# lambdaji/tf_repos

Hardware: NVIDIA H100
Metric: DeepFM training samples/sec, Criteo-39-field synthetic (39 fields, 200M vocab, k=16, bs=8192) (higher is better)
Workload: dtype f32

## Files before the change

include/ctr_b200.h:

```cpp
#ifndef CTR_B200_H_
#define CTR_B200_H_

#include <stddef.h>
#include <stdint.h>

#ifdef __cplusplus
extern "C" {
#endif

typedef void* ctr_stream_t;

enum ctr_status {
  CTR_OK = 0,
  CTR_ERR_INVALID_ARG = -1,
  CTR_ERR_UNSUPPORTED = -2,
  CTR_ERR_CUDA = -3,
  CTR_ERR_WORKSPACE = -4
};

enum ctr_fm_mode {
  CTR_FM_DEEPFM = 0,
  CTR_FM_NFM = 1,
  CTR_FM_PLAIN = 2
};
// ... 65 lines not shown
int ctr_epoch_sweep(int opt, float* var, float* slot0, float* slot1, uint8_t* last, int64_t n_rows, int K,
                    const float* hyper, const float* lr_table, int from, int upto, int reset, double* ss_partials,
                    int* n_partials_host, int32_t* list, int64_t list_cap, int32_t* list_count, double* ss_rows,
                    ctr_stream_t stream);
int ctr_epoch_sweep_ovf(int opt, float* var, float* slot0, float* slot1, uint8_t* last, int64_t n_rows, int K,
                        const float* hyper, const float* lr_table, int from, int upto, int reset, double* ss_partials,
                        int* n_partials_host, int32_t* list, int64_t list_cap, int32_t* list_count, double* ss_rows,
                        int32_t* list_overflow, ctr_stream_t stream);
int ctr_epoch_sweep2_supported(int opt, int64_t n_rows, int K);
int ctr_epoch_sweep2(int opt, float* var, float* slot0, float* slot1, float* w_var, float* w_slot0, float* w_slot1,
                     uint8_t* last, int64_t n_rows, int K, const float* hyper, const float* lr_table, int from, int upto,
                     int reset, double* ss_partials, double* w_ss_partials, int* n_partials_host, int32_t* list,
                     int64_t list_cap, int32_t* list_count, double* ss_rows, double* w_ss_rows, int32_t* list_overflow,
                     ctr_stream_t stream);
int ctr_epoch_reg_loss(double* ss_rows, const double* ss_partials, int n_partials, int upto, float scale,
                       float* reg, int accumulate, ctr_stream_t stream);
int ctr_selftest_divsqrt(uint64_t seed, int64_t n, int64_t* mismatches, ctr_stream_t stream);
int ctr_selftest_adam_packed(int regime, uint64_t seed, int64_t n, int steps, float lr, float l2, int64_t* out3,
                             ctr_stream_t stream);

int ctr_logit_loss(const float* bias, const float* y_a, const float* y_b, const float* y_c,
                   const float* labels, int B, int B_total, float* y, float* pred, float* loss_ce,
                   float* dy, float* dbias, ctr_stream_t stream);

int ctr_fc_fwd(const float* in, const float* Wt, const float* b, const float* drop_mask, float keep_prob,
               int M, int Kd, int Nd, int act, float* out, ctr_stream_t stream);
int ctr_fc_fwd_grouped(const float* in, const float* Wt, const float* b, const float* group_bias, int group_P,
                       const float* drop_mask, float keep_prob, int M, int Kd, int Nd, int act, float* out,
                       ctr_stream_t stream);
size_t ctr_fc_bwd_workspace_bytes(int M, int Kd, int Nd);
int ctr_fc_bwd(const float* in, const float* Wt, const float* out, const float* drop_mask, float keep_prob,
               float* dOut, int M, int Kd, int Nd, int act, float* dIn, int accumulate_din, float* dW, float* db,
               void* ws, size_t ws_bytes, ctr_stream_t stream);
int ctr_fc1_fwd(const float* in_a, int Ka, const float* in_b, int Kb, const float* w, const float* b, int M,
                float* y, ctr_stream_t stream);
size_t ctr_fc1_bwd_workspace_bytes(int M, int Ka, int Kb);
int ctr_fc1_bwd(const float* in_a, int Ka, const float* in_b, int Kb, const float* w, const float* dy, int M,
                float* d_a, float* d_b, float* dw, float* db, void* ws, size_t ws_bytes, ctr_stream_t stream);
int ctr_dropout_mask(float* mask, int64_t n, float keep_prob, uint64_t seed, const float* step_dev,
                     ctr_stream_t stream);

size_t ctr_bn_workspace_bytes(int H);
int ctr_bn_fwd(const float* x, int n, int H, const float* gamma, const float* beta, float* moving_mean,
               float* moving_var, int train, float decay, float eps, const float* drop_mask, float keep_prob, float* out,
               float* save_mean, float* save_var, void* ws, size_t ws_bytes, ctr_stream_t stream);
int ctr_bn_bwd(const float* d_out, const float* x, int n, int H, const float* save_mean, const float* save_var,
               const float* gamma, float eps, const float* drop_mask, float keep_prob, float* d_x, float* d_gamma,
               float* d_beta, void* ws, size_t ws_bytes, ctr_stream_t stream);

int ctr_cross_fwd(const float* x0, const float* w, const float* b, int B, int D, int L, float* xL, float* s,
                  ctr_stream_t stream);
size_t ctr_cross_bwd_workspace_bytes(int B, int D, int L);
int ctr_cross_bwd(const float* x0, const float* w, const float* b, const float* s, const float* dxL,
                  const float* dx_in, int B, int D, int L, float* dx0, float* dw, float* db, void* ws,
                  size_t ws_bytes, ctr_stream_t stream);

int ctr_mvm_fwd(const float* x, const float* mvm_b, int B, int F, int K, float* x_mvm, ctr_stream_t stream);
size_t ctr_mvm_bwd_workspace_bytes(int B, int F, int K);
int ctr_mvm_bwd(const float* x, const float* mvm_b, const float* d_xmvm, const float* dX, int B, int F, int K,
                float* d_e, float* d_mvm_b, void* ws, size_t ws_bytes, ctr_stream_t stream);

int ctr_esmm_embed_fwd(const int32_t* feat_ids, const int32_t* a_ids, const int32_t* bag_ids, const float* bag_wgt,
                       const int32_t* bag_off, const float* V, int64_t N, int B, int Fp, int K, float* x, int32_t* oob,
                       ctr_stream_t stream);
int ctr_esmm_embed_bwd(const float* dx, const float* bag_wgt, const int32_t* bag_off, int B, int Fp, int K,
                       int64_t n_rows, float* g_rows, ctr_stream_t stream);
// ... 145 lines not shown
```

tf_repos_b200/_lib.py:

```python
from __future__ import annotations

import ctypes
import os
from ctypes import c_char_p, c_float, c_int, c_int32, c_int64, c_size_t, c_uint64, c_void_p

_HERE = os.path.dirname(os.path.abspath(__file__))
LIB_PATH = os.path.join(_HERE, "libctr_b200.so")


class CtrError(RuntimeError):
    pass


def _load() -> ctypes.CDLL:
    if not os.path.exists(LIB_PATH):
        raise CtrError(
            f"{LIB_PATH} not found: build it with `make` (or `python -c 'import __graft_entry__ as g; "
            "g.build()'`). There is no CPU/eager fallback for the hot path."
        )
    return ctypes.CDLL(LIB_PATH)


_lib = _load()

# ... 7 lines not shown
    "ctr_fm_embed_bwd": (c_int, [P, P, P, P, P, P, c_int, c_int, c_int, c_int, P, P, P]),
    "ctr_unique_segment_workspace_bytes": (c_size_t, [c_int64, c_int64]),
    "ctr_unique_segment": (c_int, [P, c_int64, c_int64, P, P, P, P, P, P, P, c_size_t, P]),
    "ctr_segment_sum_rows": (c_int, [P, P, P, P, P, P, c_int64, c_int, P, P, P, c_size_t, P]),
    "ctr_opt_sparse_rows": (c_int, [c_int, P, P, P, P, P, P, c_int64, c_int, P, P, P]),
    "ctr_opt_dense_sweep": (c_int, [c_int, P, P, P, c_int64, P, P, ctypes.POINTER(c_int), P]),
    "ctr_opt_patch_rows": (c_int, [P, P, P, P, P, P, c_int64, c_int, c_int, P]),
    "ctr_opt_dense_grad": (c_int, [c_int, P, P, P, P, c_int64, P, P]),
    "ctr_adam_tick": (c_int, [P, P, c_int, P]),
    "ctr_epoch_max_steps": (c_int, []),
    "ctr_epoch_tick": (c_int, [P, P, c_int, P, c_int, c_int, P]),
    "ctr_epoch_rows": (c_int, [c_int, c_int, P, P, P, P, P, P, P, c_int64, c_int, P, P, c_int, P, P]),
    "ctr_epoch_rows2": (c_int, [c_int, c_int, P, P, P, P, P, P, P, P, P, P, P, P, c_int64, c_int, P, P, c_int, P, P, P]),
    "ctr_epoch_rows2_staged": (c_int, [c_int, c_int, P, P, P, P, P, P, P, P, P, P, P, P, c_int64, c_int, P, P, c_int, P,
                                       P, P, P, P]),
    "ctr_epoch_sweep": (c_int, [c_int, P, P, P, P, c_int64, c_int, P, P, c_int, c_int, c_int, P,
                                ctypes.POINTER(c_int), P, c_int64, P, P, P]),
    "ctr_epoch_sweep_ovf": (c_int, [c_int, P, P, P, P, c_int64, c_int, P, P, c_int, c_int, c_int, P,
                                    ctypes.POINTER(c_int), P, c_int64, P, P, P, P]),
    "ctr_epoch_sweep2_supported": (c_int, [c_int, c_int64, c_int]),
    "ctr_epoch_sweep2": (c_int, [c_int, P, P, P, P, P, P, P, c_int64, c_int, P, P, c_int, c_int, c_int, P, P,
                                 ctypes.POINTER(c_int), P, c_int64, P, P, P, P, P]),
    "ctr_epoch_reg_loss": (c_int, [P, P, c_int, c_int, c_float, P, c_int, P]),
    "ctr_selftest_divsqrt": (c_int, [c_uint64, c_int64, P, P]),
    "ctr_selftest_adam_packed": (c_int, [c_int, c_uint64, c_int64, c_int, c_float, c_float, P, P]),
    "ctr_reduce_sum": (c_int, [P, c_int64, c_float, P, P, c_size_t, P]),
    "ctr_l2_loss_workspace_bytes": (c_size_t, [c_int64]),
    "ctr_l2_loss": (c_int, [P, c_int64, c_float, P, P, c_size_t, P]),
    "ctr_logit_loss": (c_int, [P, P, P, P, P, c_int, c_int, P, P, P, P, P, P]),
    "ctr_fc_fwd": (c_int, [P, P, P, P, c_float, c_int, c_int, c_int, c_int, P, P]),
    "ctr_fc_bwd_workspace_bytes": (c_size_t, [c_int, c_int, c_int]),
    "ctr_fc_fwd_grouped": (c_int, [P, P, P, P, c_int, P, c_float, c_int, c_int, c_int, c_int, P, P]),
    "ctr_fc_bwd": (c_int, [P, P, P, P, c_float, P, c_int, c_int, c_int, c_int, P, c_int, P, P, P, c_size_t, P]),
    "ctr_fc1_fwd": (c_int, [P, c_int, P, c_int, P, P, c_int, P, P]),
    "ctr_fc1_bwd_workspace_bytes": (c_size_t, [c_int, c_int, c_int]),
    "ctr_fc1_bwd": (c_int, [P, c_int, P, c_int, P, P, c_int, P, P, P, P, P, c_size_t, P]),
    "ctr_dropout_mask": (c_int, [P, c_int64, c_float, c_uint64, P, P]),
    "ctr_bn_workspace_bytes": (c_size_t, [c_int]),
    "ctr_bn_fwd": (c_int, [P, c_int, c_int, P, P, P, P, c_int, c_float, c_float, P, c_float, P, P, P, P, c_size_t, P]),
    "ctr_bn_bwd": (c_int, [P, P, c_int, c_int, P, P, P, c_float, P, c_float, P, P, P, P, c_size_t, P]),
    "ctr_cross_fwd": (c_int, [P, P, P, c_int, c_int, c_int, P, P, P]),
    "ctr_cross_bwd_workspace_bytes": (c_size_t, [c_int, c_int, c_int]),
    "ctr_cross_bwd": (c_int, [P, P, P, P, P, P, c_int, c_int, c_int, P, P, P, P, c_size_t, P]),
    "ctr_mvm_fwd": (c_int, [P, P, c_int, c_int, c_int, P, P]),
    "ctr_mvm_bwd_workspace_bytes": (c_size_t, [c_int, c_int, c_int]),
    "ctr_mvm_bwd": (c_int, [P, P, P, P, c_int, c_int, c_int, P, P, P, c_size_t, P]),
    "ctr_esmm_embed_fwd": (c_int, [P, P, P, P, P, P, c_int64, c_int, c_int, c_int, P, P, P]),
    "ctr_esmm_embed_bwd": (c_int, [P, P, P, c_int, c_int, c_int, c_int64, P, P]),
    "ctr_esmm_head": (c_int, [P, P, P, P, c_int, c_int, c_float, c_float, P, P, P, P, P, P, P]),
    "ctr_gather_scale_rows": (c_int, [P, P, P, c_int64, c_int64, c_int, c_int, c_int64, P, P, P]),
    "ctr_bag_sum_fwd": (c_int, [P, P, P, P, c_int64, c_int, c_int, c_int64, P, P]),
    "ctr_bag_sum_fwd_oob": (c_int, [P, P, P, P, c_int64, c_int, c_int, c_int64, P, P, P]),
    "ctr_bag_sum_bwd": (c_int, [P, c_int64, P, P, c_int, c_int, P, P]),
    "ctr_scale_rows": (c_int, [P, P, P, c_int64, c_int, c_int, c_int64, P, P]),
    "ctr_din_pool_fwd": (c_int, [P, P, P, c_int, c_int, c_int, P, P, c_int64, P]),
    "ctr_din_pool_bwd": (c_int, [P, P, P, P, c_int64, c_int, c_int, c_int, P, P, P]),
    "ctr_group_sum": (c_int, [P, c_int, c_int, c_int, P, P]),
    "ctr_din_att_dz": (c_int, [P, P, c_float, P, P, c_int, c_int, c_int, P, P, P, P]),
    "ctr_colsum_rows": (c_int, [P, c_int, c_int, c_int, P, P]),
    "ctr_axpby": (c_int, [P, c_float, P, c_float, c_int64, P, P]),
    "ctr_pnn_product_fwd": (c_int, [P, c_int, c_int, c_int, c_int, P, P]),
    "ctr_pnn_product_bwd": (c_int, [P, P, c_int, c_int, c_int, c_int, P, P]),
    "ctr_afm_pairs_fwd": (c_int, [P, c_int, c_int, c_int, P, P]),
    "ctr_afm_pairs_bwd": (c_int, [P, P, c_int, c_int, c_int, P, P]),
    "ctr_afm_pool_fwd": (c_int, [P, P, P, c_float, c_int, c_int, c_int, P, P, P]),
    "ctr_afm_pool_bwd": (c_int, [P, P, P, c_float, P, c_int, c_int, c_int, P, P, P]),
# ... 77 lines not shown
```

tf_repos_b200/base.py:

```python
from __future__ import annotations

from typing import Dict, List, Optional

import torch

from . import ops
from .engine import DenseVars, OptimizerState, SparseModel, SparseUpdater, Table


def ints(s) -> List[int]:
    return [int(t) for t in s.split(",")] if isinstance(s, str) else list(s)


def floats(s) -> List[float]:
    return [float(t) for t in s.split(",")] if isinstance(s, str) else list(s)


class CTRModel(SparseModel):
    replayed_launches = 0
    batch_norm, bn_decay = False, 0.9
    table_name = "emb"
    linear_name: Optional[str] = None

    def __init__(self, field_size: int, feature_size: int, embedding_size: int, batch_size: int,
# ... 58 lines not shown
        B = ids.shape[0]
        self.flush()
        bias, y_a, y_b, y_c = self._forward(ids, vals, train=False)
        ops.logit_loss(bias, y_a, y_b, y_c, None, B, y=self.y[:B], pred=self.pred[:B])
        return self.pred[:B]

    def train_step(self, ids: torch.Tensor, vals: torch.Tensor, labels: torch.Tensor, masks=None) -> torch.Tensor:
        B, F, K = ids.shape[0], self.F, self.K
        assert B <= self.B, "batch larger than the configured batch_size"
        assert B == self.B or self.world == 1, "partial batches are not supported under data parallelism"
        deferred = self.update_mode == "exact_deferred"
        upd = self.updater
        upd.begin_step()
        ids_u = ids.reshape(-1)
        if deferred and self.world > 1:
            import torch.distributed as dist
            dist.all_gather_into_tensor(self.ids_all, ids_u)
            ids_u = self.ids_all
        upd.catch_up(ids_u)
        bias, y_a, y_b, y_c = self._forward(ids, vals, train=True, masks=masks)
        ops.logit_loss(bias, y_a, y_b, y_c, labels, B, y=self.y[:B], pred=self.pred[:B], loss_ce=self.loss_ce,
                       dy=self.dy[:B], dbias=(self.dense.grads[self.bias_name] if self.bias_name else None),
                       B_total=B * self.world)
        self._backward(ids, vals)
        g_rows = self.g_rows[: B * F]
        g_w = self.g_w[: B * F] if self.g_w is not None else None
        if self.world > 1:
            import torch.distributed as dist
            if not deferred:
                dist.all_gather_into_tensor(self.ids_all, ids.reshape(-1))
            dist.all_gather_into_tensor(self.g_rows_all, g_rows)
            if g_w is not None:
                dist.all_gather_into_tensor(self.g_w_all, g_w)
            dist.all_reduce(self.dense.grad)
            g_rows, g_w = self.g_rows_all, (self.g_w_all if g_w is not None else None)
        upd.finish_step(self.ids_all if self.world > 1 else ids.reshape(-1), g_rows, g_w)
        dense_reg = self._dense_reg_terms()
        self.dense.apply()
        self.global_step += 1
        parts = [self.loss_ce]
        if dense_reg is not None and not self.table_reg_first:
            parts.append(dense_reg)
        if self.W is not None:
            parts.append(upd.reg[1:2])
        parts.append(upd.reg[0:1])
        if dense_reg is not None and self.table_reg_first:
            parts.append(dense_reg)
        return torch.cat(parts)

    bias_name: Optional[str] = None
    table_reg_first = False

    def train_step_graphed(self, ids: torch.Tensor, vals: torch.Tensor, labels: torch.Tensor) -> torch.Tensor:
        B = ids.shape[0]
        deferred = self.update_mode == "exact_deferred"
        ends_epoch = deferred and self.epoch_pos == self.epoch_steps - 1
        if B != self.B or self.world != 1 or ends_epoch:
            return self.train_step(ids, vals, labels)
        if not hasattr(self, "_graphs"):
            self._graphs, self._graph_out, self._graph_seen = {}, {}, {}
            self._gin = (torch.empty(self.B, self.F, dtype=torch.int32, device=self.device),
                         torch.empty(self.B, self.F, dtype=torch.float32, device=self.device),
                         torch.empty(self.B, dtype=torch.float32, device=self.device))
        for dst, src in zip(self._gin, (ids, vals, labels)):
            dst.copy_(src, non_blocking=True)
        key = (self.update_mode, self.epoch_pos if deferred else 0)
# ... 50 lines not shown
```

tf_repos_b200/csrc/fc.cu:

```cuda
#include <stdlib.h>
#include <string.h>

#include "common.cuh"

namespace ctr {

constexpr int GEMM_BK = 16;

template <int BM, int BN, int TM, int TN, bool A_RC, bool B_RC, int EPI>
__global__ void __launch_bounds__((BM / TM) * (BN / TN))
gemm_tile_kernel(const float* __restrict__ A, int lda, const float* __restrict__ B, int ldb,
                 float* __restrict__ C, int ldc, int M, int N, int R, const float* __restrict__ bias,
                 int act, const float* __restrict__ mask, float keep, const float* __restrict__ gbias,
                 int gP) {
  constexpr int NT = (BM / TM) * (BN / TN);
  __shared__ __align__(16) float As[2][GEMM_BK][BM + 4];
  __shared__ __align__(16) float Bs[2][GEMM_BK][BN + 4];
  const int tid = threadIdx.x;
  const int tx = tid % (BN / TN), ty = tid / (BN / TN);
  const int i0 = blockIdx.y * BM, j0 = blockIdx.x * BN;
  const int r_chunk = (R + gridDim.z - 1) / gridDim.z;
  const int r_begin = blockIdx.z * r_chunk;
  const int r_end = min(R, r_begin + r_chunk);

// ... 228 lines not shown
int ctr_fc_fwd_grouped(const float* in, const float* Wt, const float* b, const float* group_bias, int group_P,
                       const float* drop_mask, float keep_prob, int M, int Kd, int Nd, int act, float* out,
                       ctr_stream_t stream);

int ctr_fc_fwd(const float* in, const float* Wt, const float* b, const float* drop_mask, float keep_prob,
               int M, int Kd, int Nd, int act, float* out, ctr_stream_t stream) {
  return ctr_fc_fwd_grouped(in, Wt, b, nullptr, 1, drop_mask, keep_prob, M, Kd, Nd, act, out, stream);
}

int ctr_fc_fwd_grouped(const float* in, const float* Wt, const float* b, const float* group_bias, int group_P,
                       const float* drop_mask, float keep_prob, int M, int Kd, int Nd, int act, float* out,
                       ctr_stream_t stream) {
  CTR_REQUIRE(M >= 0 && Kd > 0 && Nd > 0 && (act == 0 || act == 1) && group_P >= 1, CTR_ERR_INVALID_ARG,
              "ctr_fc_fwd: bad shape/act");
  if (M == 0) return CTR_OK;
  CTR_REQUIRE(in && Wt && out, CTR_ERR_INVALID_ARG, "ctr_fc_fwd: null buffer");
  CTR_REQUIRE(!drop_mask || keep_prob > 0.f, CTR_ERR_INVALID_ARG, "ctr_fc_fwd: keep_prob must be > 0");
  cudaStream_t st = as_stream(stream);
  if (use_tc()) {
    tc_gemm_dispatch(0, 1, in, Kd, Wt, Nd, out, Nd, M, Nd, Kd, 1, b, act, drop_mask, keep_prob, group_bias, group_P, st);
  } else if (Nd >= 128) {
    dim3 grid((Nd + 127) / 128, (M + 63) / 64, 1);
    gemm_tile_kernel<64, 128, 4, 8, true, false, 1><<<grid, 256, 0, st>>>(in, Kd, Wt, Nd, out, Nd, M, Nd, Kd, b, act,
                                                                          drop_mask, keep_prob, group_bias, group_P);
  } else {
    dim3 grid((Nd + 63) / 64, (M + 63) / 64, 1);
    gemm_tile_kernel<64, 64, 4, 4, true, false, 1><<<grid, 256, 0, st>>>(in, Kd, Wt, Nd, out, Nd, M, Nd, Kd, b, act,
                                                                         drop_mask, keep_prob, group_bias, group_P);
  }
  CTR_LAUNCHED("ctr_fc_fwd");
  return CTR_OK;
}

size_t ctr_fc_bwd_workspace_bytes(int M, int Kd, int Nd) {
  if (M <= 0 || Kd <= 0 || Nd <= 0) return 0;
  const size_t chunks = (size_t)(M + DZ_ROWS - 1) / DZ_ROWS;
  const size_t split = 64;
  return (chunks * (size_t)Nd + split * (size_t)Kd * (size_t)Nd) * sizeof(float);
}

int ctr_fc_bwd(const float* in, const float* Wt, const float* out, const float* drop_mask, float keep_prob,
               float* dOut, int M, int Kd, int Nd, int act, float* dIn, int accumulate_din, float* dW, float* db,
               void* ws, size_t ws_bytes, ctr_stream_t stream) {
  CTR_REQUIRE(M >= 0 && Kd > 0 && Nd > 0 && (act == 0 || act == 1 || act == 2), CTR_ERR_INVALID_ARG, "ctr_fc_bwd: bad shape/act");
  if (M == 0) return CTR_OK;
  CTR_REQUIRE(in && Wt && dOut && dW && (act == 2 || (out && db)), CTR_ERR_INVALID_ARG, "ctr_fc_bwd: null buffer");
  CTR_REQUIRE(ws && ws_bytes >= ctr_fc_bwd_workspace_bytes(M, Kd, Nd), CTR_ERR_WORKSPACE,
              "ctr_fc_bwd: workspace too small");
  cudaStream_t st = as_stream(stream);
  float* colsum = reinterpret_cast<float*>(ws);
  const int chunks = (M + DZ_ROWS - 1) / DZ_ROWS;
  float* dw_part = colsum + (size_t)chunks * Nd;
  if (act != 2) {
    fc_dz_kernel<<<dim3((Nd + 31) / 32, chunks), 256, 0, st>>>(dOut, out, drop_mask, keep_prob, M, Nd, act, colsum);
    CTR_LAUNCHED("fc_dz");
    colsum_rows_kernel<<<(Nd + 31) / 32, 256, 0, st>>>(colsum, chunks, Nd, Nd, Nd, db, nullptr);
    CTR_LAUNCHED("fc_db_reduce");
  }
  const bool dw_transposed = use_tc() && Kd <= 64 && Nd >= 128;
  const int S = dw_transposed ? pick_split(Nd, Kd, M) : pick_split(Kd, Nd, M);
  if (dw_transposed) {
    tc_gemm_dispatch(2, 0, dOut, Nd, in, Kd, dw_part, Kd, Nd, Kd, M, S, nullptr, 0, nullptr, 1.f, nullptr, 1, st);
    CTR_LAUNCHED("fc_dw(t)");
    const int64_t n = (int64_t)Kd * Nd;
    splitk_reduce_t_kernel<<<(unsigned)((n + 255) / 256), 256, 0, st>>>(dw_part, S, Kd, Nd, dW);
    CTR_LAUNCHED("fc_dw_reduce(t)");
  } else {
    if (use_tc()) {
      tc_gemm_dispatch(2, 0, in, Kd, dOut, Nd, S == 1 ? dW : dw_part, Nd, Kd, Nd, M, S, nullptr, 0, nullptr, 1.f, nullptr, 1, st);
    } else {
      dim3 grid((Nd + 63) / 64, (Kd + 63) / 64, S);
      gemm_tile_kernel<64, 64, 4, 4, false, false, 0><<<grid, 256, 0, st>>>(in, Kd, dOut, Nd, S == 1 ? dW : dw_part, Nd,
                                                                            Kd, Nd, M, nullptr, 0, nullptr, 1.f, nullptr, 1);
    }
    CTR_LAUNCHED("fc_dw");
    if (S > 1) {
      const int64_t n = (int64_t)Kd * Nd;
      splitk_reduce_kernel<<<(unsigned)((n + 255) / 256), 256, 0, st>>>(dw_part, S, n, dW);
      CTR_LAUNCHED("fc_dw_reduce");
    }
  }
  if (dIn && use_tc()) {
    tc_gemm_dispatch(1, accumulate_din ? 2 : 0, dOut, Nd, Wt, Nd, dIn, Kd, M, Kd, Nd, 1, nullptr, 0, nullptr, 1.f, nullptr, 1, st);
    CTR_LAUNCHED("fc_din");
  } else if (dIn) {
    dim3 grid((Kd + 127) / 128, (M + 63) / 64, 1);
    if (accumulate_din)
      gemm_tile_kernel<64, 128, 4, 8, true, true, 2><<<grid, 256, 0, st>>>(dOut, Nd, Wt, Nd, dIn, Kd, M, Kd, Nd, nullptr,
                                                                           0, nullptr, 1.f, nullptr, 1);
    else
      gemm_tile_kernel<64, 128, 4, 8, true, true, 0><<<grid, 256, 0, st>>>(dOut, Nd, Wt, Nd, dIn, Kd, M, Kd, Nd, nullptr,
                                                                           0, nullptr, 1.f, nullptr, 1);
    CTR_LAUNCHED("fc_din");
  }
  return CTR_OK;
}

int ctr_colsum_rows(const float* part, int rows, int ld, int ncols, float* out, ctr_stream_t stream) {
  CTR_REQUIRE(rows >= 0 && ncols > 0 && ld >= ncols, CTR_ERR_INVALID_ARG, "ctr_colsum_rows: bad shape");
  CTR_REQUIRE(part && out, CTR_ERR_INVALID_ARG, "ctr_colsum_rows: null buffer");
  colsum_rows_kernel<<<(ncols + 31) / 32, 256, 0, as_stream(stream)>>>(part, rows, ld, ncols, ncols, out, nullptr);
  CTR_LAUNCHED("ctr_colsum_rows");
  return CTR_OK;
}

int ctr_fc1_fwd(const float* in_a, int Ka, const float* in_b, int Kb, const float* w, const float* b, int M,
                float* y, ctr_stream_t stream) {
  CTR_REQUIRE(M >= 0 && Ka > 0 && Kb >= 0, CTR_ERR_INVALID_ARG, "ctr_fc1_fwd: bad shape");
  if (M == 0) return CTR_OK;
  CTR_REQUIRE(in_a && w && y && (Kb == 0 || in_b), CTR_ERR_INVALID_ARG, "ctr_fc1_fwd: null buffer");
  fc1_fwd_kernel<<<(M + 7) / 8, 256, 0, as_stream(stream)>>>(in_a, Ka, in_b, Kb, w, b, M, y);
  CTR_LAUNCHED("ctr_fc1_fwd");
  return CTR_OK;
}

size_t ctr_fc1_bwd_workspace_bytes(int M, int Ka, int Kb) {
  if (M <= 0) return 0;
  return (size_t)((M + FC1_ROWS - 1) / FC1_ROWS) * (size_t)(Ka + Kb + 1) * sizeof(float);
}

int ctr_fc1_bwd(const float* in_a, int Ka, const float* in_b, int Kb, const float* w, const float* dy, int M,
                float* d_a, float* d_b, float* dw, float* db, void* ws, size_t ws_bytes, ctr_stream_t stream) {
  CTR_REQUIRE(M >= 0 && Ka > 0 && Kb >= 0, CTR_ERR_INVALID_ARG, "ctr_fc1_bwd: bad shape");
  if (M == 0) return CTR_OK;
  CTR_REQUIRE(in_a && w && dy && dw && db && (Kb == 0 || in_b), CTR_ERR_INVALID_ARG, "ctr_fc1_bwd: null buffer");
  CTR_REQUIRE(ws && ws_bytes >= ctr_fc1_bwd_workspace_bytes(M, Ka, Kb), CTR_ERR_WORKSPACE,
              "ctr_fc1_bwd: workspace too small");
  cudaStream_t st = as_stream(stream);
  const int chunks = (M + FC1_ROWS - 1) / FC1_ROWS;
  float* part = reinterpret_cast<float*>(ws);
// ... 22 lines not shown
```

tf_repos_b200/deepfm.py:

```python
from __future__ import annotations

import torch

from . import ops
from .base import CTRModel, floats, ints
from .engine import DenseVars
from .mlp import MLP


class DeepFM(CTRModel):
    table_name = "fm_v"
    linear_name = "fm_w"
    bias_name = "fm_bias"

    def __init__(self, field_size: int, feature_size: int, embedding_size: int, batch_size: int,
                 deep_layers="256,128,64", dropout="0.5,0.5,0.5", l2_reg: float = 1e-4,
                 learning_rate: float = 5e-4, optimizer: str = "Adam", update_mode: str = "exact",
                 device="cuda", seed: int = 0, world: int = 1, epoch_steps: int = 8, batch_norm: bool = False,
                 batch_norm_decay: float = 0.9):
        self.layers, self.keep = ints(deep_layers), floats(dropout)
        self.batch_norm, self.bn_decay = bool(batch_norm), float(batch_norm_decay)
        super().__init__(field_size, feature_size, embedding_size, batch_size, l2_reg, learning_rate, optimizer,
                         update_mode, device, seed, world, epoch_steps)
        self.fm_v, self.fm_w = self.V, self.W

    def _build(self):
        B, F, K, dev = self.B, self.F, self.K, self.device
        f32 = dict(dtype=torch.float32, device=dev)
        self.mlp = MLP(F * K, self.layers, self.keep, B, dev, seed=self.seed, batch_norm=self.batch_norm,
                       bn_decay=self.bn_decay)
        self.dense = DenseVars([("fm_bias", (1,))] + self.mlp.specs(), self.opt, dev)
        self.mlp.init(self.dense, torch.Generator().manual_seed(self.seed))
        self.x = torch.empty(B, F * K, **f32)
        self.S = torch.empty(B, K, **f32)
        self.y_w = torch.empty(B, **f32)
        self.y_v = torch.empty(B, **f32)
        self.d_last = torch.empty(B, self.mlp.out_in, **f32)

    def _forward(self, ids, vals, train: bool, masks=None):
        B = ids.shape[0]
        ops.fm_embed_fwd(ids, vals, self.V.var, self.W.var, ops.FM_DEEPFM, x=self.x[:B], y_w=self.y_w[:B],
                         y2=self.y_v[:B], S=self.S[:B], oob=self.oob)
        self._a = self.mlp.forward_hidden(self.x[:B], self.dense, train, masks, step_dev=self.opt.state[3:4])
        y_d = self.mlp.forward_out(self._a, self.dense)
        return self.dense["fm_bias"], self.y_w[:B], self.y_v[:B], y_d

    def _backward(self, ids, vals):
        B = ids.shape[0]
        dy = self.dy[:B]
        self.mlp.backward_out(self._a, dy, self.dense, self.d_last[:B])
        dX = self.mlp.backward_hidden(self.x[:B], self.d_last[:B], self.dense)
        ops.fm_embed_bwd(vals, self.x[:B], self.S[:B], dX, dy, dy, self.K, ops.FM_DEEPFM,
                         self.g_rows[: B * self.F], self.g_w[: B * self.F])
```

tf_repos_b200/engine.py:

```python
from __future__ import annotations

import math
from typing import Dict, List, Optional, Sequence, Tuple

import torch

from . import ops

HYPER_TABLE, HYPER_DENSE, HYPER_DENSE_L2 = 0, 1, 2


class OptimizerState:

    def __init__(self, optimizer: str, learning_rate: float, l2_reg: float, device, adagrad_init: float = 1e-8):
        self.adagrad_init = adagrad_init
        if optimizer not in ops.OPT_BY_NAME:
            raise NameError(f"optimizer {optimizer!r} is not one of {sorted(ops.OPT_BY_NAME)}")
        self.name = optimizer
        self.opt = ops.OPT_BY_NAME[optimizer]
        self.n_slots = ops.OPT_SLOTS[self.opt]
        self.device = device
        aux = (0.0, 0.0, 0.0)
        beta1, beta2, eps = 0.9, 0.999, 1e-8
        if optimizer == "Momentum":
# ... 264 lines not shown
        vs = self.variables()
        for name, v in values.items():
            vs[name].copy_(v.to(self.device, torch.float32).reshape(vs[name].shape))


class DenseVars:

    def __init__(self, specs: Sequence[Tuple[str, Tuple[int, ...]]], opt: OptimizerState, device,
                 l2_names: Sequence[str] = (), tail: int = 4):
        specs = [s for s in specs if s[0] in l2_names] + [s for s in specs if s[0] not in l2_names]
        self.opt = opt
        sizes = [int(math.prod(shape)) for _, shape in specs]
        pad = lambda x: (x + 3) // 4 * 4
        offs, o = [], 0
        for sz in sizes:
            offs.append(o)
            o += pad(sz)
        self.total = o
        self.n_l2 = sum(pad(sz) for (nm, _), sz in zip(specs, sizes) if nm in l2_names)
        f32 = dict(dtype=torch.float32, device=device)
        self.flat = torch.zeros(max(self.total, 4), **f32)
        self.grad = torch.zeros(max(self.total, 4) + tail, **f32)
        self.tail = self.grad[max(self.total, 4):]
        self.slots = []
        for s in range(opt.n_slots):
            t = torch.empty(max(self.total, 4), **f32)
            ops.fill(t, opt.slot_init(s))
            self.slots.append(t)
        self.views: Dict[str, torch.Tensor] = {}
        self.grads: Dict[str, torch.Tensor] = {}
        for (nm, shape), off, sz in zip(specs, offs, sizes):
            self.views[nm] = self.flat[off:off + sz].view(shape)
            self.grads[nm] = self.grad[off:off + sz].view(shape)

    def __getitem__(self, name):
        return self.views[name]

    def apply(self):
        o = self.opt
        s1 = lambda a, b: (self.slots[1][a:b] if o.n_slots > 1 else None)
        if self.n_l2:
            ops.opt_dense_grad(o.opt, self.flat[:self.n_l2], self.slots[0][:self.n_l2], s1(0, self.n_l2),
                               self.grad[:self.n_l2], o.record(HYPER_DENSE_L2))
        if self.total > self.n_l2:
            a, b = self.n_l2, self.total
            ops.opt_dense_grad(o.opt, self.flat[a:b], self.slots[0][a:b], s1(a, b), self.grad[a:b],
                               o.record(HYPER_DENSE))
```

tf_repos_b200/mlp.py:

```python
from __future__ import annotations

from typing import Optional, Sequence

import torch

from . import ops
from .engine import DenseVars


class MLP:

    def __init__(self, in_dim: int, layers: Sequence[int], keep_prob: Sequence[float], B: int, device,
                 scope: str = "Deep-part", out_scope: Optional[str] = "deep_out", out_extra_in: int = 0,
                 seed: int = 0, layer_fmt: str = "mlp{i}", w_name: str = "weights", b_name: str = "biases",
                 batch_norm: bool = False, bn_decay: float = 0.9, *, bn_fmt: str = "bn_{i}"):
        self.layer_fmt, self.w_name, self.b_name, self.bn_fmt = layer_fmt, w_name, b_name, bn_fmt
        self.in_dim, self.layers, self.keep = in_dim, list(layers), list(keep_prob)
        self.scope, self.out_scope, self.B, self.device = scope, out_scope, B, device
        self.out_name = out_scope if (out_scope and "/" in out_scope) else self._scoped(out_scope)
        self.last_dim = self.layers[-1] if self.layers else in_dim
        self.out_extra_in = out_extra_in
        self.out_in = self.last_dim + out_extra_in
        self.seed = seed
        f32 = dict(dtype=torch.float32, device=device)
        self.h = [torch.empty(B, w, **f32) for w in self.layers]
        self.masks = [torch.empty(B, w, **f32) if k < 1.0 else None for w, k in zip(self.layers, self.keep)]
        self.dh = [torch.empty(B, w, **f32) for w in self.layers]
        self.y = torch.empty(B, **f32)
        self.dx = torch.empty(B, in_dim, **f32)
        self.d_extra = torch.empty(B, out_extra_in, **f32) if out_extra_in else None
        self.batch_norm, self.bn_decay = bool(batch_norm), float(bn_decay)
        self.bn_state = {}
        if self.batch_norm:
            self.r = [torch.empty(B, w, **f32) for w in self.layers]
            self.dr = [torch.empty(B, w, **f32) for w in self.layers]
            self.bn_mean = [torch.zeros(w, **f32) for w in self.layers]
            self.bn_var = [torch.ones(w, **f32) for w in self.layers]
            for i, w in enumerate(self.layers):
                self.bn_state[self._bn(i, "moving_mean")] = torch.zeros(w, **f32)
                self.bn_state[self._bn(i, "moving_variance")] = torch.ones(w, **f32)
        dims = [in_dim] + self.layers
        ws = max([ops.fc_bwd_workspace_bytes(B, dims[i], dims[i + 1]) for i in range(len(self.layers))] +
                 [ops.fc1_bwd_workspace_bytes(B, self.last_dim, out_extra_in), 16])
        self.ws = torch.empty(ws, dtype=torch.uint8, device=device)
        self._active = [None] * len(self.layers)

    def _scoped(self, name: str) -> str:
        return f"{self.scope}/{name}" if self.scope else name

    def _w(self, i: int) -> str:
        return self._scoped(f"{self.layer_fmt.format(i=i)}/{self.w_name}")

    def _b(self, i: int) -> str:
        return self._scoped(f"{self.layer_fmt.format(i=i)}/{self.b_name}")

    def _bn(self, i: int, what: str) -> str:
        return self._scoped(f"{self.bn_fmt.format(i=i)}/{what}")

    def specs(self):
        out, d = [], self.in_dim
        for i, w in enumerate(self.layers):
            out += [(self._w(i), (d, w)), (self._b(i), (w,))]
            if self.batch_norm:
                out += [(self._bn(i, "gamma"), (w,)), (self._bn(i, "beta"), (w,))]
            d = w
        if self.out_scope:
            out += [(f"{self.out_name}/{self.w_name}", (self.out_in, 1)), (f"{self.out_name}/{self.b_name}", (1,))]
        return out

    def init(self, dv: DenseVars, gen: torch.Generator):
        for name, shape in self.specs():
            if name.endswith(self.w_name):
                lim = (6.0 / (shape[0] + shape[1])) ** 0.5
                w = (torch.rand(shape, generator=gen, dtype=torch.float64) * 2 - 1) * lim
                dv[name].copy_(w.to(torch.float32))
            elif name.endswith("/gamma"):
# ... 26 lines not shown
    def forward_out(self, a: torch.Tensor, dv: DenseVars, extra: Optional[torch.Tensor] = None) -> torch.Tensor:
        W, b = dv[f"{self.out_name}/{self.w_name}"], dv[f"{self.out_name}/{self.b_name}"]
        y = self.y[: a.shape[0]]
        if extra is not None:
            ops.fc1_fwd(extra, a, W.view(-1), b, y)
        else:
            ops.fc1_fwd(a, None, W.view(-1), b, y)
        return y

    def backward_out(self, a: torch.Tensor, dy: torch.Tensor, dv: DenseVars, da: torch.Tensor,
                     extra: Optional[torch.Tensor] = None):
        W = dv[f"{self.out_name}/{self.w_name}"]
        gW = dv.grads[f"{self.out_name}/{self.w_name}"].view(-1)
        gb = dv.grads[f"{self.out_name}/{self.b_name}"]
        if extra is not None:
            ops.fc1_bwd(extra, a, W.view(-1), dy, self.d_extra[: a.shape[0]], da, gW, gb, self.ws)
        else:
            ops.fc1_bwd(a, None, W.view(-1), dy, da, None, gW, gb, self.ws)

    def backward_hidden(self, x: torch.Tensor, d_last: torch.Tensor, dv: DenseVars, need_dx: bool = True):
        d = d_last
        n = d.shape[0]
        if not self.layers:
            return d_last
        for i in reversed(range(len(self.layers))):
            W = dv[self._w(i)]
            a = self.h[i - 1][:n] if i > 0 else x
            d_in = self.dh[i - 1][:n] if i > 0 else (self.dx[:n] if need_dx else None)
            if self.batch_norm:
                r, dr = self.r[i][:n], self.dr[i][:n]
                ops.bn_bwd(d, r, self.bn_mean[i], self.bn_var[i], dv[self._bn(i, "gamma")], self._active[i], self.keep[i],
                           dr, dv.grads[self._bn(i, "gamma")], dv.grads[self._bn(i, "beta")])
                ops.fc_bwd(a, W, r, None, 1.0, dr, 1, d_in, dv.grads[self._w(i)], dv.grads[self._b(i)], self.ws)
            else:
                ops.fc_bwd(a, W, self.h[i][:n], self._active[i], self.keep[i], d, 1, d_in,
                           dv.grads[self._w(i)], dv.grads[self._b(i)], self.ws)
            d = d_in
        return self.dx[:n] if need_dx else None
```

tf_repos_b200/ops.py:

```python
from __future__ import annotations

import ctypes
from typing import Optional

import torch

from . import _lib
from ._lib import CtrError, check

FM_DEEPFM, FM_NFM, FM_PLAIN = 0, 1, 2
OPT_ADAM, OPT_ADAGRAD, OPT_MOMENTUM, OPT_FTRL = 0, 1, 2, 3
OPT_BY_NAME = {"Adam": OPT_ADAM, "Adagrad": OPT_ADAGRAD, "Momentum": OPT_MOMENTUM, "ftrl": OPT_FTRL}
OPT_SLOTS = {OPT_ADAM: 2, OPT_ADAGRAD: 1, OPT_MOMENTUM: 1, OPT_FTRL: 2}
LONG_SEG = 128

_L = _lib.raw()


def _stream() -> int:
    return torch.cuda.current_stream().cuda_stream


def _p(t: Optional[torch.Tensor], dtype=None, name="tensor") -> Optional[int]:
    if t is None:
# ... 122 lines not shown
def adam_tick(state, hyper):
    check(_L.ctr_adam_tick(_p(state, torch.float32, "state"), _p(hyper, torch.float32, "hyper"),
                           hyper.numel() // 8, _stream()), "ctr_adam_tick")


def fc_fwd(inp, Wt, b, drop_mask, keep_prob, act, out):
    M, Kd = inp.shape
    Nd = Wt.shape[1]
    check(_L.ctr_fc_fwd(_p(inp, torch.float32, "in"), _p(Wt, torch.float32, "Wt"), _p(b, torch.float32, "b"),
                        _p(drop_mask, torch.float32, "drop_mask"), float(keep_prob), M, Kd, Nd, act,
                        _p(out, torch.float32, "out"), _stream()), "ctr_fc_fwd")


def fc_bwd_workspace_bytes(M, Kd, Nd) -> int:
    return int(_L.ctr_fc_bwd_workspace_bytes(M, Kd, Nd))


def fc_fwd_grouped(inp, Wt, b, group_bias, group_P, drop_mask, keep_prob, act, out):
    M, Kd = inp.shape
    Nd = Wt.shape[1]
    check(_L.ctr_fc_fwd_grouped(_p(inp, torch.float32, "in"), _p(Wt, torch.float32, "Wt"), _p(b, torch.float32, "b"),
                                _p(group_bias, torch.float32, "group_bias"), group_P,
                                _p(drop_mask, torch.float32, "drop_mask"), float(keep_prob), M, Kd, Nd, act,
                                _p(out, torch.float32, "out"), _stream()), "ctr_fc_fwd_grouped")


def fc_bwd(inp, Wt, out, drop_mask, keep_prob, dOut, act, dIn, dW, db, ws, accumulate_din=False):
    M, Kd = inp.shape
    Nd = Wt.shape[1]
    check(_L.ctr_fc_bwd(_p(inp, torch.float32, "in"), _p(Wt, torch.float32, "Wt"), _p(out, torch.float32, "out"),
                        _p(drop_mask, torch.float32, "drop_mask"), float(keep_prob), _p(dOut, torch.float32, "dOut"),
                        M, Kd, Nd, act, _p(dIn, torch.float32, "dIn"), int(accumulate_din), _p(dW, torch.float32, "dW"),
                        _p(db, torch.float32, "db"), _p(ws), ws.numel() * ws.element_size(), _stream()), "ctr_fc_bwd")


def fc1_fwd(in_a, in_b, w, b, y):
    M, Ka = in_a.shape
    Kb = in_b.shape[1] if in_b is not None else 0
    check(_L.ctr_fc1_fwd(_p(in_a, torch.float32, "in_a"), Ka, _p(in_b, torch.float32, "in_b"), Kb,
                         _p(w, torch.float32, "w"), _p(b, torch.float32, "b"), M, _p(y, torch.float32, "y"),
                         _stream()), "ctr_fc1_fwd")


def fc1_bwd_workspace_bytes(M, Ka, Kb) -> int:
    return int(_L.ctr_fc1_bwd_workspace_bytes(M, Ka, Kb))


def fc1_bwd(in_a, in_b, w, dy, d_a, d_b, dw, db, ws):
    M, Ka = in_a.shape
    Kb = in_b.shape[1] if in_b is not None else 0
    check(_L.ctr_fc1_bwd(_p(in_a, torch.float32, "in_a"), Ka, _p(in_b, torch.float32, "in_b"), Kb,
                         _p(w, torch.float32, "w"), _p(dy, torch.float32, "dy"), M, _p(d_a, torch.float32, "d_a"),
                         _p(d_b, torch.float32, "d_b"), _p(dw, torch.float32, "dw"), _p(db, torch.float32, "db"),
                         _p(ws), ws.numel() * ws.element_size(), _stream()), "ctr_fc1_bwd")


def dropout_mask(mask, keep_prob, seed, step_dev=None):
    check(_L.ctr_dropout_mask(_p(mask, torch.float32, "mask"), mask.numel(), float(keep_prob), int(seed),
                              _p(step_dev, torch.float32, "step"), _stream()), "ctr_dropout_mask")


BN_EPS = 1e-3


_bn_ws = {}

# ... 487 lines not shown
```

Measured before the change: 1.539 million.

## Split FC backward into dx and dW, run weight-gradient GEMMs on side stream

Splits the fully connected backward into a dx/bias-grad part and a separate weight-gradient part, each with its own workspace. In DeepFM without batch norm, each layer's dW GEMM and split-K reduce are forked onto a side CUDA stream, so they can overlap with the dx chain of the layers below. The dense variables record the pending stream and join it before the optimizer apply and the all-reduce. This adds stream synchronisation, an extra workspace buffer, and the risk of buffer-lifetime races across streams. The fork can be turned off with an environment variable.

```diff
diff --git a/include/ctr_b200.h b/include/ctr_b200.h
--- a/include/ctr_b200.h
+++ b/include/ctr_b200.h
@@ -121,6 +121,12 @@
 int ctr_fc_bwd(const float* in, const float* Wt, const float* out, const float* drop_mask, float keep_prob,
                float* dOut, int M, int Kd, int Nd, int act, float* dIn, int accumulate_din, float* dW, float* db,
                void* ws, size_t ws_bytes, ctr_stream_t stream);
+int ctr_fc_bwd_dx(const float* Wt, const float* out, const float* drop_mask, float keep_prob, float* dOut, int M,
+                  int Kd, int Nd, int act, float* dIn, int accumulate_din, float* db, void* ws, size_t ws_bytes,
+                  ctr_stream_t stream);
+size_t ctr_fc_bwd_dw_workspace_bytes(int M, int Kd, int Nd);
+int ctr_fc_bwd_dw(const float* in, const float* dZ, int M, int Kd, int Nd, float* dW, void* ws, size_t ws_bytes,
+                  ctr_stream_t stream);
 int ctr_fc1_fwd(const float* in_a, int Ka, const float* in_b, int Kb, const float* w, const float* b, int M,
                 float* y, ctr_stream_t stream);
 size_t ctr_fc1_bwd_workspace_bytes(int M, int Ka, int Kb);
diff --git a/tf_repos_b200/_lib.py b/tf_repos_b200/_lib.py
--- a/tf_repos_b200/_lib.py
+++ b/tf_repos_b200/_lib.py
@@ -63,6 +63,9 @@
     "ctr_fc_bwd_workspace_bytes": (c_size_t, [c_int, c_int, c_int]),
     "ctr_fc_fwd_grouped": (c_int, [P, P, P, P, c_int, P, c_float, c_int, c_int, c_int, c_int, P, P]),
     "ctr_fc_bwd": (c_int, [P, P, P, P, c_float, P, c_int, c_int, c_int, c_int, P, c_int, P, P, P, c_size_t, P]),
+    "ctr_fc_bwd_dx": (c_int, [P, P, P, c_float, P, c_int, c_int, c_int, c_int, P, c_int, P, P, c_size_t, P]),
+    "ctr_fc_bwd_dw_workspace_bytes": (c_size_t, [c_int, c_int, c_int]),
+    "ctr_fc_bwd_dw": (c_int, [P, P, c_int, c_int, c_int, P, P, c_size_t, P]),
     "ctr_fc1_fwd": (c_int, [P, c_int, P, c_int, P, P, c_int, P, P]),
     "ctr_fc1_bwd_workspace_bytes": (c_size_t, [c_int, c_int, c_int]),
     "ctr_fc1_bwd": (c_int, [P, c_int, P, c_int, P, P, c_int, P, P, P, P, P, c_size_t, P]),
diff --git a/tf_repos_b200/base.py b/tf_repos_b200/base.py
--- a/tf_repos_b200/base.py
+++ b/tf_repos_b200/base.py
@@ -114,6 +114,7 @@
             dist.all_gather_into_tensor(self.g_rows_all, g_rows)
             if g_w is not None:
                 dist.all_gather_into_tensor(self.g_w_all, g_w)
+            self.dense.join()
             dist.all_reduce(self.dense.grad)
             g_rows, g_w = self.g_rows_all, (self.g_w_all if g_w is not None else None)
         upd.finish_step(self.ids_all if self.world > 1 else ids.reshape(-1), g_rows, g_w)
diff --git a/tf_repos_b200/csrc/fc.cu b/tf_repos_b200/csrc/fc.cu
--- a/tf_repos_b200/csrc/fc.cu
+++ b/tf_repos_b200/csrc/fc.cu
@@ -284,53 +284,37 @@
   return CTR_OK;
 }
 
+static size_t fc_dz_workspace_bytes(int M, int Nd) {
+  return (size_t)((M + DZ_ROWS - 1) / DZ_ROWS) * (size_t)Nd * sizeof(float);
+}
+
+size_t ctr_fc_bwd_dw_workspace_bytes(int M, int Kd, int Nd) {
+  if (M <= 0 || Kd <= 0 || Nd <= 0) return 0;
+  const size_t split = 64;
+  return split * (size_t)Kd * (size_t)Nd * sizeof(float);
+}
+
 size_t ctr_fc_bwd_workspace_bytes(int M, int Kd, int Nd) {
   if (M <= 0 || Kd <= 0 || Nd <= 0) return 0;
-  const size_t chunks = (size_t)(M + DZ_ROWS - 1) / DZ_ROWS;
-  const size_t split = 64;
-  return (chunks * (size_t)Nd + split * (size_t)Kd * (size_t)Nd) * sizeof(float);
-}
-
-int ctr_fc_bwd(const float* in, const float* Wt, const float* out, const float* drop_mask, float keep_prob,
-               float* dOut, int M, int Kd, int Nd, int act, float* dIn, int accumulate_din, float* dW, float* db,
-               void* ws, size_t ws_bytes, ctr_stream_t stream) {
+  return fc_dz_workspace_bytes(M, Nd) + ctr_fc_bwd_dw_workspace_bytes(M, Kd, Nd);
+}
+
+int ctr_fc_bwd_dx(const float* Wt, const float* out, const float* drop_mask, float keep_prob, float* dOut, int M,
+                  int Kd, int Nd, int act, float* dIn, int accumulate_din, float* db, void* ws, size_t ws_bytes,
+                  ctr_stream_t stream) {
   CTR_REQUIRE(M >= 0 && Kd > 0 && Nd > 0 && (act == 0 || act == 1 || act == 2), CTR_ERR_INVALID_ARG, "ctr_fc_bwd: bad shape/act");
   if (M == 0) return CTR_OK;
-  CTR_REQUIRE(in && Wt && dOut && dW && (act == 2 || (out && db)), CTR_ERR_INVALID_ARG, "ctr_fc_bwd: null buffer");
-  CTR_REQUIRE(ws && ws_bytes >= ctr_fc_bwd_workspace_bytes(M, Kd, Nd), CTR_ERR_WORKSPACE,
+  CTR_REQUIRE(Wt && dOut && (act == 2 || (out && db)), CTR_ERR_INVALID_ARG, "ctr_fc_bwd: null buffer");
+  CTR_REQUIRE(act == 2 || (ws && ws_bytes >= fc_dz_workspace_bytes(M, Nd)), CTR_ERR_WORKSPACE,
               "ctr_fc_bwd: workspace too small");
   cudaStream_t st = as_stream(stream);
-  float* colsum = reinterpret_cast<float*>(ws);
-  const int chunks = (M + DZ_ROWS - 1) / DZ_ROWS;
-  float* dw_part = colsum + (size_t)chunks * Nd;
   if (act != 2) {
+    float* colsum = reinterpret_cast<float*>(ws);
+    const int chunks = (M + DZ_ROWS - 1) / DZ_ROWS;
     fc_dz_kernel<<<dim3((Nd + 31) / 32, chunks), 256, 0, st>>>(dOut, out, drop_mask, keep_prob, M, Nd, act, colsum);
     CTR_LAUNCHED("fc_dz");
     colsum_rows_kernel<<<(Nd + 31) / 32, 256, 0, st>>>(colsum, chunks, Nd, Nd, Nd, db, nullptr);
     CTR_LAUNCHED("fc_db_reduce");
-  }
-  const bool dw_transposed = use_tc() && Kd <= 64 && Nd >= 128;
-  const int S = dw_transposed ? pick_split(Nd, Kd, M) : pick_split(Kd, Nd, M);
-  if (dw_transposed) {
-    tc_gemm_dispatch(2, 0, dOut, Nd, in, Kd, dw_part, Kd, Nd, Kd, M, S, nullptr, 0, nullptr, 1.f, nullptr, 1, st);
-    CTR_LAUNCHED("fc_dw(t)");
-    const int64_t n = (int64_t)Kd * Nd;
-    splitk_reduce_t_kernel<<<(unsigned)((n + 255) / 256), 256, 0, st>>>(dw_part, S, Kd, Nd, dW);
-    CTR_LAUNCHED("fc_dw_reduce(t)");
-  } else {
-    if (use_tc()) {
-      tc_gemm_dispatch(2, 0, in, Kd, dOut, Nd, S == 1 ? dW : dw_part, Nd, Kd, Nd, M, S, nullptr, 0, nullptr, 1.f, nullptr, 1, st);
-    } else {
-      dim3 grid((Nd + 63) / 64, (Kd + 63) / 64, S);
-      gemm_tile_kernel<64, 64, 4, 4, false, false, 0><<<grid, 256, 0, st>>>(in, Kd, dOut, Nd, S == 1 ? dW : dw_part, Nd,
-                                                                            Kd, Nd, M, nullptr, 0, nullptr, 1.f, nullptr, 1);
-    }
-    CTR_LAUNCHED("fc_dw");
-    if (S > 1) {
-      const int64_t n = (int64_t)Kd * Nd;
-      splitk_reduce_kernel<<<(unsigned)((n + 255) / 256), 256, 0, st>>>(dw_part, S, n, dW);
-      CTR_LAUNCHED("fc_dw_reduce");
-    }
   }
   if (dIn && use_tc()) {
     tc_gemm_dispatch(1, accumulate_din ? 2 : 0, dOut, Nd, Wt, Nd, dIn, Kd, M, Kd, Nd, 1, nullptr, 0, nullptr, 1.f, nullptr, 1, st);
@@ -348,6 +332,56 @@
   return CTR_OK;
 }
 
+int ctr_fc_bwd_dw(const float* in, const float* dZ, int M, int Kd, int Nd, float* dW, void* ws, size_t ws_bytes,
+                  ctr_stream_t stream) {
+  CTR_REQUIRE(M >= 0 && Kd > 0 && Nd > 0, CTR_ERR_INVALID_ARG, "ctr_fc_bwd_dw: bad shape");
+  if (M == 0) return CTR_OK;
+  CTR_REQUIRE(in && dZ && dW, CTR_ERR_INVALID_ARG, "ctr_fc_bwd_dw: null buffer");
+  CTR_REQUIRE(ws && ws_bytes >= ctr_fc_bwd_dw_workspace_bytes(M, Kd, Nd), CTR_ERR_WORKSPACE,
+              "ctr_fc_bwd_dw: workspace too small");
+  cudaStream_t st = as_stream(stream);
+  float* dw_part = reinterpret_cast<float*>(ws);
+  const bool dw_transposed = use_tc() && Kd <= 64 && Nd >= 128;
+  const int S = dw_transposed ? pick_split(Nd, Kd, M) : pick_split(Kd, Nd, M);
+  if (dw_transposed) {
+    tc_gemm_dispatch(2, 0, dZ, Nd, in, Kd, dw_part, Kd, Nd, Kd, M, S, nullptr, 0, nullptr, 1.f, nullptr, 1, st);
+    CTR_LAUNCHED("fc_dw(t)");
+    const int64_t n = (int64_t)Kd * Nd;
+    splitk_reduce_t_kernel<<<(unsigned)((n + 255) / 256), 256, 0, st>>>(dw_part, S, Kd, Nd, dW);
+    CTR_LAUNCHED("fc_dw_reduce(t)");
+  } else {
+    if (use_tc()) {
+      tc_gemm_dispatch(2, 0, in, Kd, dZ, Nd, S == 1 ? dW : dw_part, Nd, Kd, Nd, M, S, nullptr, 0, nullptr, 1.f, nullptr, 1, st);
+    } else {
+      dim3 grid((Nd + 63) / 64, (Kd + 63) / 64, S);
+      gemm_tile_kernel<64, 64, 4, 4, false, false, 0><<<grid, 256, 0, st>>>(in, Kd, dZ, Nd, S == 1 ? dW : dw_part, Nd,
+                                                                            Kd, Nd, M, nullptr, 0, nullptr, 1.f, nullptr, 1);
+    }
+    CTR_LAUNCHED("fc_dw");
+    if (S > 1) {
+      const int64_t n = (int64_t)Kd * Nd;
+      splitk_reduce_kernel<<<(unsigned)((n + 255) / 256), 256, 0, st>>>(dw_part, S, n, dW);
+      CTR_LAUNCHED("fc_dw_reduce");
+    }
+  }
+  return CTR_OK;
+}
+
+int ctr_fc_bwd(const float* in, const float* Wt, const float* out, const float* drop_mask, float keep_prob,
+               float* dOut, int M, int Kd, int Nd, int act, float* dIn, int accumulate_din, float* dW, float* db,
+               void* ws, size_t ws_bytes, ctr_stream_t stream) {
+  CTR_REQUIRE(M >= 0 && Kd > 0 && Nd > 0 && (act == 0 || act == 1 || act == 2), CTR_ERR_INVALID_ARG, "ctr_fc_bwd: bad shape/act");
+  if (M == 0) return CTR_OK;
+  CTR_REQUIRE(in && Wt && dOut && dW && (act == 2 || (out && db)), CTR_ERR_INVALID_ARG, "ctr_fc_bwd: null buffer");
+  CTR_REQUIRE(ws && ws_bytes >= ctr_fc_bwd_workspace_bytes(M, Kd, Nd), CTR_ERR_WORKSPACE,
+              "ctr_fc_bwd: workspace too small");
+  const size_t dz_bytes = fc_dz_workspace_bytes(M, Nd);
+  const int rc = ctr_fc_bwd_dx(Wt, out, drop_mask, keep_prob, dOut, M, Kd, Nd, act, dIn, accumulate_din, db, ws,
+                               dz_bytes, stream);
+  if (rc != CTR_OK) return rc;
+  return ctr_fc_bwd_dw(in, dOut, M, Kd, Nd, dW, static_cast<uint8_t*>(ws) + dz_bytes, ws_bytes - dz_bytes, stream);
+}
+
 int ctr_colsum_rows(const float* part, int rows, int ld, int ncols, float* out, ctr_stream_t stream) {
   CTR_REQUIRE(rows >= 0 && ncols > 0 && ld >= ncols, CTR_ERR_INVALID_ARG, "ctr_colsum_rows: bad shape");
   CTR_REQUIRE(part && out, CTR_ERR_INVALID_ARG, "ctr_colsum_rows: null buffer");
diff --git a/tf_repos_b200/deepfm.py b/tf_repos_b200/deepfm.py
--- a/tf_repos_b200/deepfm.py
+++ b/tf_repos_b200/deepfm.py
@@ -28,7 +28,7 @@
         B, F, K, dev = self.B, self.F, self.K, self.device
         f32 = dict(dtype=torch.float32, device=dev)
         self.mlp = MLP(F * K, self.layers, self.keep, B, dev, seed=self.seed, batch_norm=self.batch_norm,
-                       bn_decay=self.bn_decay)
+                       bn_decay=self.bn_decay, fork_dw=True)
         self.dense = DenseVars([("fm_bias", (1,))] + self.mlp.specs(), self.opt, dev)
         self.mlp.init(self.dense, torch.Generator().manual_seed(self.seed))
         self.x = torch.empty(B, F * K, **f32)
diff --git a/tf_repos_b200/engine.py b/tf_repos_b200/engine.py
--- a/tf_repos_b200/engine.py
+++ b/tf_repos_b200/engine.py
@@ -320,11 +320,23 @@
         for (nm, shape), off, sz in zip(specs, offs, sizes):
             self.views[nm] = self.flat[off:off + sz].view(shape)
             self.grads[nm] = self.grad[off:off + sz].view(shape)
+        self._pending: List[torch.cuda.Stream] = []
 
     def __getitem__(self, name):
         return self.views[name]
 
+    def defer(self, stream: torch.cuda.Stream):
+        if stream not in self._pending:
+            self._pending.append(stream)
+
+    def join(self):
+        cur = torch.cuda.current_stream()
+        for s in self._pending:
+            cur.wait_stream(s)
+        self._pending.clear()
+
     def apply(self):
+        self.join()
         o = self.opt
         s1 = lambda a, b: (self.slots[1][a:b] if o.n_slots > 1 else None)
         if self.n_l2:
diff --git a/tf_repos_b200/mlp.py b/tf_repos_b200/mlp.py
--- a/tf_repos_b200/mlp.py
+++ b/tf_repos_b200/mlp.py
@@ -1,5 +1,6 @@
 from __future__ import annotations
 
+import os
 from typing import Optional, Sequence
 
 import torch
@@ -13,7 +14,7 @@
     def __init__(self, in_dim: int, layers: Sequence[int], keep_prob: Sequence[float], B: int, device,
                  scope: str = "Deep-part", out_scope: Optional[str] = "deep_out", out_extra_in: int = 0,
                  seed: int = 0, layer_fmt: str = "mlp{i}", w_name: str = "weights", b_name: str = "biases",
-                 batch_norm: bool = False, bn_decay: float = 0.9, *, bn_fmt: str = "bn_{i}"):
+                 batch_norm: bool = False, bn_decay: float = 0.9, *, bn_fmt: str = "bn_{i}", fork_dw: bool = False):
         self.layer_fmt, self.w_name, self.b_name, self.bn_fmt = layer_fmt, w_name, b_name, bn_fmt
         self.in_dim, self.layers, self.keep = in_dim, list(layers), list(keep_prob)
         self.scope, self.out_scope, self.B, self.device = scope, out_scope, B, device
@@ -40,8 +41,17 @@
                 self.bn_state[self._bn(i, "moving_mean")] = torch.zeros(w, **f32)
                 self.bn_state[self._bn(i, "moving_variance")] = torch.ones(w, **f32)
         dims = [in_dim] + self.layers
-        ws = max([ops.fc_bwd_workspace_bytes(B, dims[i], dims[i + 1]) for i in range(len(self.layers))] +
-                 [ops.fc1_bwd_workspace_bytes(B, self.last_dim, out_extra_in), 16])
+        self.fork = (fork_dw and not self.batch_norm and bool(self.layers) and torch.device(device).type == "cuda"
+                     and _fork_enabled())
+        if self.fork:
+            ws = max([ops.fc_bwd_workspace_bytes(B, dims[i], dims[i + 1]) - ops.fc_bwd_dw_workspace_bytes(B, dims[i], dims[i + 1])
+                      for i in range(len(self.layers))] + [ops.fc1_bwd_workspace_bytes(B, self.last_dim, out_extra_in), 16])
+            ws_dw = max(ops.fc_bwd_dw_workspace_bytes(B, dims[i], dims[i + 1]) for i in range(len(self.layers)))
+            self.ws_dw = torch.empty(ws_dw, dtype=torch.uint8, device=device)
+            self.side = torch.cuda.Stream(device=device)
+        else:
+            ws = max([ops.fc_bwd_workspace_bytes(B, dims[i], dims[i + 1]) for i in range(len(self.layers))] +
+                     [ops.fc1_bwd_workspace_bytes(B, self.last_dim, out_extra_in), 16])
         self.ws = torch.empty(ws, dtype=torch.uint8, device=device)
         self._active = [None] * len(self.layers)
 
@@ -134,8 +144,27 @@
                 ops.bn_bwd(d, r, self.bn_mean[i], self.bn_var[i], dv[self._bn(i, "gamma")], self._active[i], self.keep[i],
                            dr, dv.grads[self._bn(i, "gamma")], dv.grads[self._bn(i, "beta")])
                 ops.fc_bwd(a, W, r, None, 1.0, dr, 1, d_in, dv.grads[self._w(i)], dv.grads[self._b(i)], self.ws)
+            elif self.fork:
+                ops.fc_bwd_dx(W, self.h[i][:n], self._active[i], self.keep[i], d, 1, d_in, dv.grads[self._b(i)], self.ws)
+                self._fork_dw(a, d, dv.grads[self._w(i)], dv)
             else:
                 ops.fc_bwd(a, W, self.h[i][:n], self._active[i], self.keep[i], d, 1, d_in,
                            dv.grads[self._w(i)], dv.grads[self._b(i)], self.ws)
             d = d_in
         return self.dx[:n] if need_dx else None
+
+    def _fork_dw(self, a: torch.Tensor, dz: torch.Tensor, gW: torch.Tensor, dv: DenseVars):
+        self.side.wait_stream(torch.cuda.current_stream())
+        with torch.cuda.stream(self.side):
+            ops.fc_bwd_dw(a, dz, gW, self.ws_dw)
+        dv.defer(self.side)
+
+
+_FORK = None
+
+
+def _fork_enabled() -> bool:
+    global _FORK
+    if _FORK is None:
+        _FORK = os.environ.get("CTR_MLP_FORK", "1") != "0"
+    return _FORK
diff --git a/tf_repos_b200/ops.py b/tf_repos_b200/ops.py
--- a/tf_repos_b200/ops.py
+++ b/tf_repos_b200/ops.py
@@ -178,6 +178,26 @@
                         _p(drop_mask, torch.float32, "drop_mask"), float(keep_prob), _p(dOut, torch.float32, "dOut"),
                         M, Kd, Nd, act, _p(dIn, torch.float32, "dIn"), int(accumulate_din), _p(dW, torch.float32, "dW"),
                         _p(db, torch.float32, "db"), _p(ws), ws.numel() * ws.element_size(), _stream()), "ctr_fc_bwd")
+
+
+def fc_bwd_dx(Wt, out, drop_mask, keep_prob, dOut, act, dIn, db, ws, accumulate_din=False):
+    M, Nd = dOut.shape
+    Kd = Wt.shape[0]
+    check(_L.ctr_fc_bwd_dx(_p(Wt, torch.float32, "Wt"), _p(out, torch.float32, "out"),
+                           _p(drop_mask, torch.float32, "drop_mask"), float(keep_prob), _p(dOut, torch.float32, "dOut"),
+                           M, Kd, Nd, act, _p(dIn, torch.float32, "dIn"), int(accumulate_din), _p(db, torch.float32, "db"),
+                           _p(ws), ws.numel() * ws.element_size(), _stream()), "ctr_fc_bwd_dx")
+
+
+def fc_bwd_dw_workspace_bytes(M, Kd, Nd) -> int:
+    return int(_L.ctr_fc_bwd_dw_workspace_bytes(M, Kd, Nd))
+
+
+def fc_bwd_dw(inp, dZ, dW, ws):
+    M, Kd = inp.shape
+    Nd = dZ.shape[1]
+    check(_L.ctr_fc_bwd_dw(_p(inp, torch.float32, "in"), _p(dZ, torch.float32, "dZ"), M, Kd, Nd,
+                           _p(dW, torch.float32, "dW"), _p(ws), ws.numel() * ws.element_size(), _stream()), "ctr_fc_bwd_dw")
 
 
 def fc1_fwd(in_a, in_b, w, b, y):
```

Result: no change. 1.554 million (median of 6 runs) (+0.9%).
